# Yelp/nrtsearch

Measured on NVIDIA H100. Metric: BM25 queries/sec (batch 1024, 10M docs), higher is better.
Workload: dtype f32

## Files before the change

### nrtsearch_b200/csrc/probe_kernel.cuh

```cuda
#pragma once
#include "query_eval.cuh"
#include "sort_kernel.cuh"
#include "collect_kernel.cuh"

namespace nrtgpu {
namespace v3 {

__device__ __forceinline__ uint32_t smem_u32(const void* p) { return (uint32_t)__cvta_generic_to_shared(p); }
__device__ __forceinline__ void mbar_init(uint64_t* bar, uint32_t count) {
  asm volatile("mbarrier.init.shared::cta.b64 [%0], %1;" ::"r"(smem_u32(bar)), "r"(count) : "memory");
}
__device__ __forceinline__ void mbar_arrive_expect_tx(uint64_t* bar, uint32_t bytes) {
  asm volatile("mbarrier.arrive.expect_tx.shared::cta.b64 _, [%0], %1;" ::"r"(smem_u32(bar)), "r"(bytes) : "memory");
}
__device__ __forceinline__ bool mbar_try_wait(uint64_t* bar, uint32_t parity) {
  uint32_t ok;
  asm volatile(
      "{\n\t.reg .pred p;\n\tmbarrier.try_wait.parity.shared::cta.b64 p, [%1], %2;\n\tselp.u32 %0, 1, 0, p;\n\t}"
      : "=r"(ok) : "r"(smem_u32(bar)), "r"(parity) : "memory");
  return ok != 0;
}
__device__ __forceinline__ void bulk_g2s(void* dst, const void* src, uint32_t bytes, uint64_t* bar) {
  asm volatile("cp.async.bulk.shared::cluster.global.mbarrier::complete_tx::bytes [%0], [%1], %2, [%3];" ::"r"(smem_u32(dst)),
               "l"(src), "r"(bytes), "r"(smem_u32(bar)) : "memory");
}

__device__ __forceinline__ uint32_t presence4(uint32_t s) {
  return ((s & 0xffu) ? 1u : 0u) | ((s & 0xff00u) ? 2u : 0u) | ((s & 0xff0000u) ? 4u : 0u) | ((s & 0xff000000u) ? 8u : 0u);
}

__device__ __forceinline__ uint32_t expand4(uint32_t m) {
  return ((m & 1u) ? 0xffu : 0u) | ((m & 2u) ? 0xff00u : 0u) | ((m & 4u) ? 0xff0000u : 0u) | ((m & 8u) ? 0xff000000u : 0u);
}

#ifdef NRT_PROBE_KNOCK
#define NRT_KNOCK(bit) ((L.knock & (bit)) != 0)
#else
#define NRT_KNOCK(bit) false
#endif
constexpr int kStageA = 8192;
constexpr int kCtasB = 4, kStageB = 6656;
constexpr int kThreads = 256;
constexpr int kAlign = 16;
constexpr int kPostingPad = 1024;
constexpr int kLongReserve = kT * (kGran + 2 * kAlign);
#ifndef NRT_PROBE_R
#define NRT_PROBE_R 2
#endif
constexpr int kR = NRT_PROBE_R;
constexpr int kCand = 1024;
static_assert(kProbeMaxTopK == kCand / 2, "the probe kernel keeps top_k <= half its candidate buffer");
constexpr int kUbt = 4 * 4 * 4 * 4;
static_assert(sizeof(DevProbeQuery::ubt) == kUbt * sizeof(float), "one bound per tf pattern");
constexpr int kWq = 32 * kR;
constexpr int kProbeStats = 31;
constexpr uint32_t kPiece = 8192;
constexpr uint32_t kTfInexact = 0xFEu;

enum { kAbsent = 0, kLong = 1, kShort = 2, kPlane = 3, kGlobal = 4 };

struct ProbeLaunch {
  DevIndexView ix;
  const DevProbeQuery* pquery;
  const int32_t* work_query;
  const int32_t* work_slice;
  const uint32_t* sbounds;
  unsigned int* work_counter;
  unsigned long long* stats;
  int32_t n_work, n_lists, n_slices, top_k;
  int32_t parts_max;
  int32_t slice_docs;
  int32_t n_gran;
  int64_t threshold;
  int32_t* pruned;
  uint64_t* theta;
  unsigned long long* total_hits;
  uint64_t* slice_keys;
  int32_t* slice_cnt;
  long long deadline_ns;
  unsigned long long* clock0;
  int32_t* timed_out;
  long long terminate_after;
  int32_t* terminated;
  int32_t sort_kind, sort_reverse;
  const uint32_t* sort_codes;
  const uint32_t* sort_missing_code;
  const AggLaunch* aggs;
  const unsigned long long* known_hits;
  int32_t knock;
};

template <int kStageT>
struct alignas(128) ProbeSmemT {
  static constexpr int kStage = kStageT;
  static constexpr int kShortMax = kStageT - kLongReserve;
  static_assert(kShortMax >= 1024, "stage too small");
  int32_t sdocs[kStageT];
  uint8_t sf8[kStageT];
  uint32_t gb[kT][kMaxSliceGran + 4];
  uint64_t cand[kCand];
  uint2 wq[kThreads / 32][kWq];
  DevProbeQuery pq;
  uint64_t stage_bar;
  uint32_t s_ia[kT], s_ib[kT];
  uint32_t s_ra[kT], s_rb[kT];
  int32_t s_sdelta[kT];
  uint32_t s_need[kT];
  uint32_t s_candbelow[kT];
  uint32_t s_cntbefore[kT];
  uint32_t s_pre[kT + 1];
  uint32_t drv_mask, ess_mask, plane_mask, long_mask, short_mask, global_mask;
  int32_t short_total;
  int32_t g1;
  int32_t run_d0, run_d1;
  int32_t staged;
  int wi;
  int skip;
  int cand_count;
  unsigned long long hits0;
  unsigned long long hits_known;
  int theta_dec;
  unsigned long long theta;
  int dbg_theta0;
  int32_t warm_g;
  uint32_t warm_own;
  uint32_t s_candrun[kT], s_cntrun[kT];
  uint32_t run_drv;
};
static_assert(sizeof(ProbeSmemT<kStageA>) <= 232448 / kCtasA - 1024 && sizeof(ProbeSmemT<kStageB>) <= 232448 / kCtasB - 1024, "ProbeSmem exceeds the per-CTA shared memory budget");

__device__ __forceinline__ int32_t seg_first(uint32_t a, uint32_t pbm) { return (int32_t)((a + pbm) & ~(uint32_t)(kAlign - 1)) - (int32_t)pbm; }
__device__ __forceinline__ uint32_t seg_n(uint32_t a, uint32_t b, uint32_t pbm) {
  return b > a ? ((b + pbm + kAlign - 1) & ~(uint32_t)(kAlign - 1)) - ((a + pbm) & ~(uint32_t)(kAlign - 1)) : 0u;
}

template <typename SM>
__device__ __noinline__ bool evaluate_doc(const ProbeLaunch& L, const SM& sm, int32_t doc, uint32_t word, float* out_score) {
  int cur_field = -1;
  uint32_t nb = 1u;
  auto term = [&](const DevClause& c, float* s) {
    uint32_t b = (word >> (8 * c.slot)) & 0xffu;
    if (b == 0) return false;
    if (c.scoring) {
      if (b == kTfInexact && sm.pq.plane[c.slot]) b = (uint32_t)__ldg(sm.pq.plane[c.slot] + doc);
      if (c.field != cur_field) {
        cur_field = c.field;
        const uint8_t* nrm = L.ix.norms[c.field];
        nb = nrm ? (uint32_t)__ldg(nrm + doc) : 1u;
      }
      const float f = (b == 255u) ? exact_freq_slow(L.ix, c, doc) : (float)b;
      *s = bm25_score(c.weight, f, __ldg(&L.ix.caches[c.field * 256 + nb]));
    }
    return true;
  };
  return eval_clauses(L.ix, sm.pq.q, sm.pq.cl, doc, presence4(word), term, out_score);
}

template <typename SM>
__device__ __forceinline__ float score_disjunction(const ProbeLaunch& L, const SM& sm, const uint8_t* norms0, int n_term,
                                                   int32_t doc, uint32_t word) {
  const uint32_t nb = norms0 ? (uint32_t)__ldg(norms0 + doc) : 1u;
  double sum = 0.0;
#pragma unroll
  for (int s = 0; s < kT; ++s) {
    if (s >= n_term) break;
    uint32_t b = (word >> (8 * s)) & 0xffu;
    if (b == 0) continue;
    if (b == kTfInexact && sm.pq.plane[s]) b = (uint32_t)__ldg(sm.pq.plane[s] + doc);
    const float f = (b == 255u) ? exact_freq_slow(L.ix, sm.pq.cl[sm.pq.clause[s]], doc) : (float)b;
    sum += (double)bm25_score(sm.pq.weight[s], f, __ldg(&L.ix.caches[sm.pq.field[s] * 256 + nb]));
  }
  return (float)sum;
}

template <typename SM>
__device__ __noinline__ void flush_candidates(const ProbeLaunch& L, SM& sm, int top_k, uint64_t* g_theta) {
  const long long ts = L.stats ? clock64() : 0ll;
  flush_top_k(sm.cand, sm.cand_count, kCand, top_k, (unsigned long long)sm.theta_dec, g_theta, sm.theta);
  if (L.stats && threadIdx.x == 0) atomicAdd(&L.stats[15], (unsigned long long)(clock64() - ts));
}

template <typename SM>
__device__ __forceinline__ uint32_t probe_smem(const SM& sm, int l, int h, int32_t doc) {
  const int end = h;
  while (l < h) {
    const int mid = (l + h) >> 1;
    if (sm.sdocs[mid] < doc) l = mid + 1; else h = mid;
  }
  return (l < end && sm.sdocs[l] == doc) ? (uint32_t)sm.sf8[l] : 0u;
}
__device__ __noinline__ uint32_t probe_global(const int32_t* docs, const uint8_t* f8, uint32_t l, uint32_t h, int32_t doc) {
  const uint32_t end = h;
  while (l < h) {
    const uint32_t mid = (l + h) >> 1;
    if (__ldg(docs + mid) < doc) l = mid + 1; else h = mid;
  }
  return (l < end && __ldg(docs + l) == doc) ? (uint32_t)__ldg(f8 + l) : 0u;
}

__device__ __forceinline__ uint32_t maxscore_nonessential(const DevProbeQuery& pq, int n_term, unsigned long long theta, bool complete,
                                                          const unsigned long long& hits_known, int64_t threshold) {
  uint32_t ne = 0;
  if (theta != 0ull && (complete || (int64_t)hits_known > threshold)) {
    const float theta_s = key_score(theta);
    for (int a = 0; a < n_term; ++a) {
      if (!(pq.pre[a] < theta_s)) break;
      ne |= 1u << pq.ord[a];
    }
  }
  return ne;
}

template <typename SM>
__device__ __noinline__ void count_role_stats(const ProbeLaunch& L, const SM& sm, int qi, int slice, uint32_t ess_mask,
                                              unsigned long long cyc, unsigned long long driver_postings) {
  const int n_term = sm.pq.q.n_term;
  const uint32_t all = (1u << n_term) - 1u;
  const bool complete = L.threshold >= (int64_t)INT32_MAX;
  const unsigned long long theta = *(volatile unsigned long long*)&L.theta[qi];
  const unsigned long long hits = *(volatile unsigned long long*)&L.total_hits[qi];
  const unsigned long long hits_known = hits > sm.hits_known ? hits : sm.hits_known;
  const uint32_t ne0 = all & ~ess_mask;
  const uint32_t ne1 = maxscore_nonessential(sm.pq, n_term, theta > sm.theta ? theta : sm.theta, complete, hits_known, L.threshold);
  if (sm.dbg_theta0) atomicAdd(&L.stats[19], cyc);
  if ((ne1 & ne0) == ne0 && ne1 != ne0) {
    unsigned long long turned = 0;
    for (int s = 0; s < n_term; ++s) if (((ne1 & ~ne0) >> s) & 1u) turned += sm.s_ib[s] - sm.s_ia[s];
    atomicAdd(&L.stats[22], 1ull); atomicAdd(&L.stats[23], cyc); atomicAdd(&L.stats[24], driver_postings); atomicAdd(&L.stats[25], turned);
    if (slice <= 1) atomicAdd(&L.stats[26 + slice], 1ull);
  }
}

template <bool kSimple, bool kStats, int kCtas, int kStageT, bool kMulti = false>
__global__ void __launch_bounds__(kThreads, kCtas) posting_probe_kernel(const __grid_constant__ ProbeLaunch L) {
  extern __shared__ __align__(128) unsigned char smem_raw[];
  using ProbeSmem = ProbeSmemT<kStageT>;
  constexpr int kStage = kStageT, kShortMax = ProbeSmem::kShortMax;
  ProbeSmem& sm = *reinterpret_cast<ProbeSmem*>(smem_raw);
  const int tid = threadIdx.x;
  const int lane = tid & 31;
  if (tid == 0) {
    mbar_init(&sm.stage_bar, 1);
    asm volatile("fence.mbarrier_init.release.cluster;" ::: "memory");
    asm volatile("fence.proxy.async.shared::cta;" ::: "memory");
  }
  uint32_t stage_parity = 0;
  const int gran_per_slice = L.slice_docs >> kLogGran;
  const int fine = (gran_per_slice + L.parts_max - 1) / L.parts_max;
  const int sb_stride = boundary_entries(L.n_slices, L.parts_max);
  const long long t_cta = kStats ? clock64() : 0ll;

  for (;;) {
    __syncthreads();
    if (tid == 0) {
      const int w = (int)atomicAdd(L.work_counter, 1u);
      sm.wi = w;
      sm.skip = 0;
      if (L.deadline_ns && w < L.n_work && deadline_passed(L.deadline_ns, L.clock0)) {
        sm.skip = 1; L.timed_out[L.work_query[w]] = 1;
      }
    }
    __syncthreads();
    const int wi = sm.wi;
    if (wi >= L.n_work) break;
    if (sm.skip) continue;
    const long long t_start = kStats ? clock64() : 0ll;
    const int qi = L.work_query[wi];
    const int32_t item = L.work_slice[wi];
    const int slice = item_slice(item);
    const int wflags = item_flags(item);
    const bool sweep_warm = (wflags & kItemSweep) != 0;
    const int warm_slot = item_sweep_slot(item);
    const int g_first = slice * gran_per_slice;
    const int g_count = min(gran_per_slice, L.n_gran - g_first);
    const ItemSpan span = item_span(item, g_count, fine, L.parts_max, L.n_slices);
    const int g_lo = span.g_lo, g_hi = span.g_hi;
    {
      constexpr int n16 = (int)((kSimple ? sizeof(DevProbeQuery) : offsetof(DevProbeQuery, ubt)) / 16);
      static_assert(n16 <= kThreads && kThreads == 64 * kT, "one 16-byte piece per thread; 64 threads per slot's granule offsets");
      constexpr int kGbIter = (kMaxSliceGran + 1 + 63) / 64;
      const int gs = tid >> 6, gj = g_lo + (tid & 63);
      const int gran_row = sweep_warm ? -1 : __ldg(&L.pquery[qi].row[gs]);
      uint4 piece = make_uint4(0u, 0u, 0u, 0u);
      if (tid < n16) piece = __ldg(reinterpret_cast<const uint4*>(L.pquery + qi) + tid);
      unsigned long long theta = 0ull, hits0 = 0ull, known = 0ull;
      uint32_t ba = 0, bb = 0, bw = 0, bx = 0;
      int exact_slot = -1;
      if (tid == 0) {
        theta = *(volatile unsigned long long*)&L.theta[qi];
        hits0 = *(volatile unsigned long long*)&L.total_hits[qi];
        if (L.known_hits) known = L.known_hits[qi];
      }
      if (tid >= 32 && tid < 32 + kT) {
        const uint32_t* sb = L.sbounds + ((size_t)qi * kT + (tid - 32)) * sb_stride;
        ba = sb[span.e_lo];
        bb = sb[span.e_hi];
        if (wflags & kItemBehindWarm) bw = sb[boundary_warm_entry(L.n_slices, L.parts_max)];
        if (kSimple && sweep_warm) { exact_slot = __ldg(&L.pquery[qi].warm_slot); bx = sb[boundary_exact_entry(L.n_slices, L.parts_max)]; }
      }
      uint32_t gv[kGbIter];
      const uint32_t* row = L.ix.gran_tab + (size_t)max(gran_row, 0) * (size_t)(L.n_gran + 1) + g_first;
#pragma unroll
      for (int k = 0; k < kGbIter; ++k) gv[k] = (gran_row >= 0 && gj + 64 * k <= g_hi) ? __ldg(row + gj + 64 * k) : 0u;
      if (tid < n16) reinterpret_cast<uint4*>(&sm.pq)[tid] = piece;
      if (tid == 0) {
        sm.cand_count = 0;
        sm.theta = theta; sm.hits0 = hits0; sm.hits_known = known > hits0 ? known : hits0;
        sm.theta_dec = sweep_warm ? 1 : 0;
      }
      if (tid >= 32 && tid < 32 + kT) {
        const int s = tid - 32;
        const uint32_t a = max(ba, bw);
        if (sweep_warm && s == warm_slot) bb = (s == exact_slot) ? bx : min(bb, a + kSweepPostings);
        sm.s_ia[s] = a; sm.s_ib[s] = max(a, bb); sm.s_ra[s] = 0; sm.s_rb[s] = 0; sm.s_sdelta[s] = 0;
      }
#pragma unroll
      for (int k = 0; k < kGbIter; ++k) if (gran_row >= 0 && gj + 64 * k <= g_hi) sm.gb[gs][gj + 64 * k] = gv[k];
    }
    __syncthreads();
    if (L.terminate_after > 0 && (long long)sm.hits0 >= L.terminate_after) {
      if (tid == 0) L.terminated[qi] = 1;
      continue;
    }
    const int n_term = sm.pq.q.n_term;
    if (tid < kT) {
      const int t = tid;
      const uint32_t all = (n_term >= 32) ? 0xffffffffu : ((1u << n_term) - 1u);
      const bool complete = L.threshold >= (int64_t)INT32_MAX;
      const uint32_t ne = (kSimple && !sweep_warm) ? maxscore_nonessential(sm.pq, n_term, sm.theta, complete, sm.hits_known, L.threshold) : 0u;
      uint32_t pm = 0;
      for (int s = 0; s < n_term; ++s) if (sm.pq.kind[s] == kPlane) pm |= 1u << s;
      uint32_t drv, ess;
      int cnt_first = -1;
      const bool exact_warm = kSimple && sm.pq.warm_slot >= 0;
      if (kSimple && sweep_warm) {
        drv = ess = 1u << warm_slot;
        if (t < n_term) { sm.s_candbelow[t] = 0u; sm.s_cntbefore[t] = exact_warm ? 0u : 0xffffffffu; sm.s_need[t] = pm & ~(1u << t); }
      } else if (kSimple) {
        ess = all & ~ne;
        if (complete && ne && !L.ix.live_bits) {
          uint32_t best = 0;
          for (int s = 0; s < n_term; ++s)
            if (((ne & pm) >> s) & 1u) { const uint32_t n = sm.s_ib[s] - sm.s_ia[s]; if (n >= best) { best = n; cnt_first = s; } }
        }
        drv = complete ? (cnt_first >= 0 ? all & ~(1u << cnt_first) : all) : ess;
        if (t < n_term) {
          const uint32_t lower = (1u << t) - 1u;
          const uint32_t first = cnt_first >= 0 ? 1u << cnt_first : 0u;
          const uint32_t below_ess = expand4(ess & lower);
          const uint32_t before_cnt = expand4((lower | first) & ~(1u << t));
          sm.s_candbelow[t] = below_ess;
          sm.s_cntbefore[t] = complete ? before_cnt : below_ess;
          sm.s_need[t] = (complete && !((ess >> t) & 1u)) ? ((lower | first) & ~(1u << t)) : (all & ~(1u << t));
        }
      } else {
        ess = sm.pq.q.dense_driver ? 0u : (sm.pq.q.driver_mask & all);
        drv = ess;
        if (t < n_term) {
          const uint32_t below = expand4(drv & ((1u << t) - 1u));
          sm.s_candbelow[t] = below; sm.s_cntbefore[t] = below;
          sm.s_need[t] = all & ~(1u << t);
        }
      }
      __syncwarp((1u << kT) - 1u);
      if (sweep_warm) {
        if (sm.pq.kind[t] != kPlane && t != warm_slot) sm.pq.kind[t] = kAbsent;
        sm.pq.row[t] = -1;
      }
      __syncwarp((1u << kT) - 1u);
      if (t == 0) {
        if (ne && !complete) L.pruned[qi] = 1;
        if (kSimple) {
          if (exact_warm && sweep_warm) sm.theta_dec = 0;
          const int warm_g = (exact_warm && !sweep_warm) ? sm.pq.warm_gran - g_first : 0;
          sm.warm_g = warm_g;
          sm.warm_own = exact_warm ? 0xffu << (8 * sm.pq.warm_slot) : 0u;
          if (exact_warm && !sweep_warm && warm_g >= g_hi) drv &= ~(1u << sm.pq.warm_slot);
        }
        int st = 0;
        uint32_t lm = 0, shm = 0, gm = 0;
        for (int s = 0; s < n_term; ++s) {
          const int k = sm.pq.kind[s];
          if (k == kLong) lm |= 1u << s;
          else if (k == kShort) {
            const uint32_t a = sm.s_ia[s], b = sm.s_ib[s];
            const int need = (int)seg_n(a, b, sm.pq.pbm[s]);
            if (st + need <= kShortMax) { sm.s_sdelta[s] = st - seg_first(a, sm.pq.pbm[s]); st += need; shm |= 1u << s; }
            else { sm.pq.kind[s] = kGlobal; gm |= 1u << s; }
          }
        }
        if (sweep_warm) { st = 0; lm = 0; shm = 0; gm = 0; }
        sm.short_total = st;
        sm.plane_mask = pm; sm.long_mask = lm; sm.short_mask = shm; sm.global_mask = gm;
        if (cnt_first >= 0 && g_lo < g_hi)
          atomicAdd(&L.total_hits[qi], (unsigned long long)(sm.s_ib[cnt_first] - sm.s_ia[cnt_first]));
        sm.drv_mask = drv; sm.ess_mask = ess;
        if (kStats) {
          sm.dbg_theta0 = kSimple && !sweep_warm && sm.theta == 0ull;
          if (sm.dbg_theta0) { atomicAdd(&L.stats[18], 1ull); if (slice <= 1) atomicAdd(&L.stats[20 + slice], 1ull); }
        }
      }
    }
    __syncthreads();

    const int32_t slice_base = slice * L.slice_docs;
    const uint32_t drv_mask = sm.drv_mask, ess_mask = sm.ess_mask;
    const uint32_t plane_mask = sm.plane_mask, long_mask = sm.long_mask, short_mask = sm.short_mask, global_mask = sm.global_mask;
    unsigned int my_hits = 0;
    unsigned long long dbg_post = 0; unsigned int dbg_runs = 0, dbg_rounds = 0, dbg_flush = 0, dbg_staged = 0, dbg_queued = 0, dbg_admit = 0;
    long long dbg_tflush = 0, dbg_twait = 0;
    const long long t_setup = kStats ? clock64() : 0ll;

    const bool dense = !kSimple && sm.pq.q.dense_driver != 0;
    const uint32_t* live = L.ix.live_bits;
    const uint32_t sort_missing = (!kSimple && L.sort_kind == NRTGPU_SORT_COLUMN) ? *L.sort_missing_code : 0u;
    int g0 = g_lo;
    if (drv_mask == 0u && !dense) g0 = g_hi;
    bool first_run = true;
    while (g0 < g_hi) {
      if (tid == 0) {
        { const unsigned long long g = *(volatile unsigned long long*)&L.theta[qi]; if (g > sm.theta) sm.theta = g; }
        const int cap = kStage - sm.short_total;
        auto fits = [&](int g1) {
          int tot = 0;
#pragma unroll
          for (int s = 0; s < kT; ++s)
            if ((long_mask >> s) & 1u) tot += (int)seg_n(sm.gb[s][g0], sm.gb[s][g1], sm.pq.pbm[s]);
          return tot <= cap;
        };
        int hi = g_hi, lo = g0 + 1;
        uint32_t run_drv = drv_mask;
        if (kSimple) {
          if (g0 < sm.warm_g && sm.warm_g < hi) hi = sm.warm_g;
          const uint32_t own = g0 < sm.warm_g ? sm.warm_own : 0u;
          for (int s = 0; s < kT; ++s) { sm.s_candrun[s] = sm.s_candbelow[s] | own; sm.s_cntrun[s] = sm.s_cntbefore[s] | own; }
          run_drv &= ~presence4(own);
          sm.run_drv = run_drv;
        }
        if (long_mask && hi > lo && !fits(hi)) {
          while (hi - lo > 1) { const int mid = (lo + hi) >> 1; if (fits(mid)) lo = mid; else hi = mid; }
          hi = lo;
        }
        const int g1 = hi;
        sm.g1 = g1;
        const bool whole = (g0 == g_lo && g1 == g_hi);
        const int32_t d0 = slice_base + (g0 << kLogGran);
        const int64_t d1_64 = (int64_t)slice_base + ((int64_t)g1 << kLogGran);
        const int32_t d1 = d1_64 > (int64_t)L.ix.n_docs ? L.ix.n_docs : (int32_t)d1_64;
        sm.run_d0 = d0; sm.run_d1 = d1;
        for (int s = 0; s < n_term; ++s) {
          const int k = sm.pq.kind[s];
          uint32_t a = sm.s_ia[s], b = sm.s_ib[s];
          if (sm.pq.row[s] >= 0) { a = max(a, sm.gb[s][g0]); b = min(b, sm.gb[s][g1]); }
          else if (!whole && b > a) {
            if (k == kShort) {
              if (!first_run) {
                const int base = sm.s_sdelta[s];
                int l = base + (int)a, h = base + (int)b;
                while (l < h) { const int m = (l + h) >> 1; if (sm.sdocs[m] < d0) l = m + 1; else h = m; }
                const uint32_t na = (uint32_t)(l - base);
                h = base + (int)b;
                while (l < h) { const int m = (l + h) >> 1; if (sm.sdocs[m] < d1) l = m + 1; else h = m; }
                a = na; b = (uint32_t)(l - base);
              }
            } else {
              const int32_t* gd = sm.pq.gdocs[s];
              uint32_t l = a, h = b;
              while (l < h) { const uint32_t m = (l + h) >> 1; if (__ldg(gd + m) < d0) l = m + 1; else h = m; }
              const uint32_t na = l;
              h = b;
              while (l < h) { const uint32_t m = (l + h) >> 1; if (__ldg(gd + m) < d1) l = m + 1; else h = m; }
              a = na; b = l;
            }
          }
          if (b < a) b = a;
          sm.s_ra[s] = a; sm.s_rb[s] = b;
        }
        uint32_t total = 0;
        if (first_run)
          for (int s = 0; s < n_term; ++s)
            if ((short_mask >> s) & 1u) total += seg_n(sm.s_ia[s], sm.s_ib[s], sm.pq.pbm[s]) * 5u;
        for (int s = 0; s < n_term; ++s)
          if ((long_mask >> s) & 1u) total += seg_n(sm.s_ra[s], sm.s_rb[s], sm.pq.pbm[s]) * 5u;
        sm.staged = total != 0u;
        if (total) {
          asm volatile("fence.proxy.async.shared::cta;" ::: "memory");
          mbar_arrive_expect_tx(&sm.stage_bar, total);
          auto stage = [&](int s, uint32_t a, uint32_t b, int at) {
            const uint32_t pbm = sm.pq.pbm[s];
            const int32_t f = seg_first(a, pbm);
            const uint32_t n = seg_n(a, b, pbm);
            sm.s_sdelta[s] = at - f;
            const unsigned char* gd = reinterpret_cast<const unsigned char*>(sm.pq.gdocs[s] + f);
            const unsigned char* gf = reinterpret_cast<const unsigned char*>(sm.pq.gf8[s] + f);
            unsigned char* dd = reinterpret_cast<unsigned char*>(&sm.sdocs[at]);
            unsigned char* df = reinterpret_cast<unsigned char*>(&sm.sf8[at]);
            for (uint32_t o = 0; o < n * 4u; o += kPiece) bulk_g2s(dd + o, gd + o, min(kPiece, n * 4u - o), &sm.stage_bar);
            for (uint32_t o = 0; o < n; o += kPiece) bulk_g2s(df + o, gf + o, min(kPiece, n - o), &sm.stage_bar);
            return (int)n;
          };
          if (first_run)
            for (int s = 0; s < n_term; ++s)
              if (((short_mask >> s) & 1u) && sm.s_ib[s] > sm.s_ia[s])
                stage(s, sm.s_ia[s], sm.s_ib[s], sm.s_sdelta[s] + seg_first(sm.s_ia[s], sm.pq.pbm[s]));
          int st = sm.short_total;
          for (int s = 0; s < n_term; ++s)
            if (((long_mask >> s) & 1u) && sm.s_rb[s] > sm.s_ra[s]) st += stage(s, sm.s_ra[s], sm.s_rb[s], st);
        }
        uint32_t pre = 0;
        for (int s = 0; s < kT; ++s) { sm.s_pre[s] = pre; if (s < n_term && ((run_drv >> s) & 1u)) pre += sm.s_rb[s] - sm.s_ra[s]; }
        sm.s_pre[kT] = pre;
      }
      __syncthreads();
      const int g1 = sm.g1;
      if (sm.staged) {
        const long long tw = kStats ? clock64() : 0ll;
        while (!mbar_try_wait(&sm.stage_bar, stage_parity)) {}
        stage_parity ^= 1u;
        if (kStats) dbg_twait += clock64() - tw;
      }
      if (first_run && g1 < g_hi && short_mask) {
        __syncthreads();
        if (tid == 0) {
          const int32_t d0 = slice_base + (g0 << kLogGran);
          const int64_t d1_64 = (int64_t)slice_base + ((int64_t)g1 << kLogGran);
          const int32_t d1 = d1_64 > (int64_t)L.ix.n_docs ? L.ix.n_docs : (int32_t)d1_64;
          for (int s = 0; s < n_term; ++s)
            if (((short_mask >> s) & 1u) && sm.s_ib[s] > sm.s_ia[s]) {
              const int base = sm.s_sdelta[s];
              int l = base + (int)sm.s_ia[s], h = base + (int)sm.s_ib[s];
              while (l < h) { const int m = (l + h) >> 1; if (sm.sdocs[m] < d0) l = m + 1; else h = m; }
              const uint32_t na = (uint32_t)(l - base);
              h = base + (int)sm.s_ib[s];
              while (l < h) { const int m = (l + h) >> 1; if (sm.sdocs[m] < d1) l = m + 1; else h = m; }
              sm.s_ra[s] = na; sm.s_rb[s] = (uint32_t)(l - base);
            }
          uint32_t pre = 0;
          for (int s = 0; s < kT; ++s) { sm.s_pre[s] = pre; if (s < n_term && (((kSimple ? sm.run_drv : drv_mask) >> s) & 1u)) pre += sm.s_rb[s] - sm.s_ra[s]; }
          sm.s_pre[kT] = pre;
        }
        __syncthreads();
      }
      if (kStats) ++dbg_runs;
      const uint32_t n_total = sm.s_pre[kT];
      if (kStats && tid == 0) { dbg_post += n_total; dbg_staged += sm.staged ? 1u : 0u; }
      int ct = 0;
      uint32_t cb = 0;
      uint64_t park = 0ull;
      bool parked = false;
      uint2* const wq = sm.wq[tid >> 5];
      int qn = 0;
      const uint32_t q_req = sm.pq.q.req_term_mask, q_not = sm.pq.q.not_term_mask;
      auto drain = [&](int n_take) -> bool {
        __syncwarp();
        bool fail = false;
        const bool have = lane < n_take;
        const uint2 e = have ? wq[qn - n_take + lane] : make_uint2(0u, 0u);
        qn -= n_take;
        const int32_t d = (int32_t)e.x;
        uint64_t entry = 0ull;
        if (kSimple) {
          if (have) {
            const uint8_t* norms0 = sm.pq.q.single_field >= 0 ? L.ix.norms[sm.pq.q.single_field] : nullptr;
            entry = make_key(score_disjunction(L, sm, norms0, n_term, d, e.y), d);
          }
        } else {
          float score;
          if (have && evaluate_doc(L, sm, d, e.y, &score)) {
            ++my_hits;
            if (L.aggs) agg_collect<kMulti>(*L.aggs, L.ix, qi, d, score);
            if (L.sort_kind == NRTGPU_SORT_RELEVANCE || L.sort_kind == kSortScoreRank) {
              entry = make_key(score, d);
              if (L.sort_kind == kSortScoreRank) entry = make_key(L.sort_reverse ? -score : score, (int32_t)__ldg(L.sort_codes + d));
            } else {
              uint32_t code = 0;
              if (L.sort_kind == NRTGPU_SORT_COLUMN) { code = __ldg(L.sort_codes + d); if (code == 0u) code = sort_missing; }
              entry = ((uint64_t)sort_hi(L.sort_kind, L.sort_reverse, code, d) << 32) | (uint32_t)(~(uint32_t)d);
            }
          }
        }
        const unsigned long long th = sm.theta;
        if (entry > th && !(sm.pq.q.has_after && !(entry < sm.pq.q.after_key)) && !NRT_KNOCK(4)) {
          if (kStats) ++dbg_admit;
          const int p = atomicAdd(&sm.cand_count, 1);
          if (p < kCand) sm.cand[p] = entry;
          else { park = entry; parked = true; fail = true; }
        }
        __syncwarp();
        return fail;
      };
      for (;;) {
        bool full = false;
        if (parked) {
          const int p = atomicAdd(&sm.cand_count, 1);
          if (p < kCand) { sm.cand[p] = park; parked = false; } else full = true;
        }
        full = __any_sync(0xffffffffu, full);
        while (!full && qn >= 32) full = __any_sync(0xffffffffu, drain(32));
        const int ct_end = NRT_KNOCK(8) ? 0 : (dense ? n_term + 1 : n_term);
        while (!full && ct < ct_end) {
          const bool t_dense = ct == n_term;
          const uint32_t n_t = t_dense ? (uint32_t)(sm.run_d1 - sm.run_d0) : ((((kSimple ? sm.run_drv : drv_mask) >> ct) & 1u) ? sm.s_rb[ct] - sm.s_ra[ct] : 0u);
          if (cb >= n_t) { ++ct; cb = 0; continue; }
          const int t = t_dense ? 0 : ct;
          const uint32_t need = t_dense ? ((n_term >= 32) ? 0xffffffffu : ((1u << n_term) - 1u)) : sm.s_need[t];
          const uint32_t need_plane = NRT_KNOCK(1) ? 0u : need & plane_mask, need_long = NRT_KNOCK(2) ? 0u : need & long_mask,
                         need_short = NRT_KNOCK(2) ? 0u : need & short_mask, need_glob = need & global_mask;
          const bool t_staged = !t_dense && (((long_mask | short_mask) >> t) & 1u);
          const bool t_ess = (ess_mask >> t) & 1u;
          const uint32_t candbelow = t_dense ? 0u : (kSimple ? sm.s_candrun[t] : sm.s_candbelow[t]),
                         cntbefore = t_dense ? 0u : (kSimple ? sm.s_cntrun[t] : sm.s_cntbefore[t]);
          const int32_t dense_d0 = sm.run_d0;
          const int32_t* sdoc_t = sm.sdocs + ((int)sm.s_ra[t] + sm.s_sdelta[t]);
          const uint8_t* sf8_t = sm.sf8 + ((int)sm.s_ra[t] + sm.s_sdelta[t]);
          const int32_t* gdoc_t = sm.pq.gdocs[t] + sm.s_ra[t];
          const uint8_t* gf8_t = sm.pq.gf8[t] + sm.s_ra[t];
          const uint32_t tshift = t_dense ? 0u : 8u * (uint32_t)t;
          const int32_t* dptr = t_staged ? sdoc_t : gdoc_t;
          const uint8_t* fptr = t_staged ? sf8_t : gf8_t;
          int32_t nd[kR]; uint32_t nf[kR];
#pragma unroll
          for (int j = 0; j < kR; ++j) {
            const uint32_t x = cb + (uint32_t)(j * kThreads + tid);
            nd[j] = -1; nf[j] = 0;
            if (x < n_t) {
              if (t_dense) nd[j] = dense_d0 + (int32_t)x; else { nd[j] = dptr[x]; nf[j] = fptr[x]; }
            }
          }
          while (!full && cb < n_t) {
            const unsigned long long theta = sm.theta;
            const float theta_s = theta ? key_score(theta) : -INFINITY;
            int32_t doc[kR]; uint32_t word[kR];
            uint32_t pbyte[kR][kT];
#pragma unroll
            for (int j = 0; j < kR; ++j) { doc[j] = nd[j]; word[j] = nf[j] << tshift; }
#pragma unroll
            for (int j = 0; j < kR; ++j) {
              const uint32_t d4 = (uint32_t)max(doc[j], 0) >> 2;
              pbyte[j][0] = 0u; pbyte[j][1] = 0u; pbyte[j][2] = 0u; pbyte[j][3] = 0u;
              if (need_plane & 1u) pbyte[j][0] = (uint32_t)__ldg(sm.pq.plane2[0] + d4);
              if (need_plane & 2u) pbyte[j][1] = (uint32_t)__ldg(sm.pq.plane2[1] + d4);
              if (need_plane & 4u) pbyte[j][2] = (uint32_t)__ldg(sm.pq.plane2[2] + d4);
              if (need_plane & 8u) pbyte[j][3] = (uint32_t)__ldg(sm.pq.plane2[3] + d4);
            }
            {
              const uint32_t nb = cb + (uint32_t)(kR * kThreads);
#pragma unroll
              for (int j = 0; j < kR; ++j) {
                const uint32_t x = nb + (uint32_t)(j * kThreads + tid);
                nd[j] = -1; nf[j] = 0;
                if (x < n_t) {
                  if (t_dense) nd[j] = dense_d0 + (int32_t)x; else { nd[j] = dptr[x]; nf[j] = fptr[x]; }
                }
              }
            }
            if (need_long | need_short | need_glob) {
#pragma unroll
              for (int j = 0; j < kR; ++j) {
                if (doc[j] < 0) continue;
                const int g = (doc[j] - slice_base) >> kLogGran;
#pragma unroll
                for (int u = 0; u < kT; ++u) {
                  uint32_t b = 0;
                  if ((need_long >> u) & 1u) {
                    const uint32_t lo = max(sm.gb[u][g], sm.s_ra[u]), hi = min(sm.gb[u][g + 1], sm.s_rb[u]);
                    if (hi > lo) b = probe_smem(sm, (int)lo + sm.s_sdelta[u], (int)hi + sm.s_sdelta[u], doc[j]);
                  } else if ((need_short >> u) & 1u) {
                    if (sm.s_rb[u] > sm.s_ra[u]) b = probe_smem(sm, (int)sm.s_ra[u] + sm.s_sdelta[u], (int)sm.s_rb[u] + sm.s_sdelta[u], doc[j]);
                  } else if ((need_glob >> u) & 1u) {
                    if (sm.s_rb[u] > sm.s_ra[u]) b = probe_global(sm.pq.gdocs[u], sm.pq.gf8[u], sm.s_ra[u], sm.s_rb[u], doc[j]);
                  }
                  word[j] |= b << (8 * u);
                }
              }
            }
            uint32_t surv_mask = 0;
#pragma unroll
            for (int j = 0; j < kR; ++j) {
              uint32_t v = word[j];
              if (need_plane) {
                const uint32_t raw = pbyte[j][0] | (pbyte[j][1] << 8) | (pbyte[j][2] << 16) | (pbyte[j][3] << 24);
                const uint32_t codes = (raw >> (((uint32_t)max(doc[j], 0) & 3u) * 2u)) & 0x03030303u;
                const uint32_t sat = __vcmpeq4(codes, 0x03030303u);
                v |= (codes & ~sat) | (sat & (kTfInexact * 0x01010101u));
              }
              bool surv = false;
              if (kSimple) {
                if (doc[j] >= 0 && !(live && !((live[doc[j] >> 5] >> (doc[j] & 31)) & 1u))) {
                  if ((v & cntbefore) == 0u) ++my_hits;
                  surv = t_ess && (v & candbelow) == 0u && !(sm.pq.ubt[__dp4a(__vminu4(v, 0x03030303u), 0x40100401u, 0u)] < theta_s);
                }
              } else {
                const uint32_t pres = presence4(v);
                surv = doc[j] >= 0 && (v & candbelow) == 0u && (pres & q_req) == q_req && (pres & q_not) == 0u;
              }
              word[j] = v;
              surv_mask |= surv ? 1u << j : 0u;
            }
#pragma unroll
            for (int j = 0; j < kR; ++j) {
              const bool surv = (surv_mask >> j) & 1u;
              const unsigned bal = __ballot_sync(0xffffffffu, surv);
              if (surv) wq[qn + __popc(bal & ((1u << lane) - 1u))] = make_uint2((uint32_t)doc[j], word[j]);
              qn += __popc(bal);
              if (kStats && lane == 0) dbg_queued += __popc(bal);
              while (!full && qn >= 32) full = __any_sync(0xffffffffu, drain(32));
            }
            cb += kR * kThreads;
            if (kStats && tid == 0) ++dbg_rounds;
          }
        }
        while (!full && qn > 0) full = __any_sync(0xffffffffu, drain(min(qn, 32)));
        __syncthreads();
        if (sm.cand_count <= kCand) break;
        const long long tf = kStats ? clock64() : 0ll;
        flush_candidates(L, sm, L.top_k, &L.theta[qi]);
        if (kStats) dbg_tflush += clock64() - tf;
        if (kStats) ++dbg_flush;
      }
      g0 = g1;
      first_run = false;
      __syncthreads();
    }

    __syncthreads();
    if (sm.cand_count > L.top_k) {
      const long long tf = kStats ? clock64() : 0ll;
      flush_candidates(L, sm, L.top_k, &L.theta[qi]);
      if (kStats) dbg_tflush += clock64() - tf;
      if (kStats) ++dbg_flush;
    }
    const bool lb_warm = kSimple ? sm.theta_dec != 0 : sweep_warm;
    const int keep = lb_warm ? 0 : min(sm.cand_count, L.top_k);
    const int out_list = item_out_list(item, L.parts_max, L.n_lists);
    uint64_t* out = L.slice_keys + ((size_t)qi * L.n_lists + out_list) * L.top_k;
    for (int i = tid; i < keep; i += kThreads) out[i] = sm.cand[i];
    if (tid == 0) L.slice_cnt[(size_t)qi * L.n_lists + out_list] = keep;
    for (int o = 16; o > 0; o >>= 1) my_hits += __shfl_xor_sync(0xffffffffu, my_hits, o);
    if (lane == 0 && my_hits && !lb_warm) atomicAdd(&L.total_hits[qi], (unsigned long long)my_hits);
    if (kStats) {
      for (int o = 16; o > 0; o >>= 1) dbg_admit += __shfl_xor_sync(0xffffffffu, dbg_admit, o);
      if (lane == 0) { atomicAdd(&L.stats[16], (unsigned long long)dbg_queued); atomicAdd(&L.stats[17], (unsigned long long)dbg_admit); }
    }
    if (kStats && tid == 0) {
      const unsigned long long cyc = (unsigned long long)(clock64() - t_start);
      atomicAdd(&L.stats[0], 1ull);
      atomicAdd(&L.stats[1], cyc);
      atomicAdd(&L.stats[2], (unsigned long long)dbg_runs);
      atomicAdd(&L.stats[3], dbg_post);
      atomicAdd(&L.stats[4], (unsigned long long)dbg_flush);
      atomicAdd(&L.stats[5], (unsigned long long)dbg_staged);
      atomicAdd(&L.stats[6], (unsigned long long)(t_setup - t_start));
      atomicAdd(&L.stats[7], (unsigned long long)dbg_rounds);
      atomicMax(&L.stats[8], cyc);
      if (wflags & (kItemWarmDocs | kItemSweep)) { atomicAdd(&L.stats[11], 1ull); atomicAdd(&L.stats[12], cyc); }
      if (sweep_warm && !lb_warm) { atomicAdd(&L.stats[28], 1ull); atomicAdd(&L.stats[29], dbg_post); atomicAdd(&L.stats[30], cyc); }
      atomicAdd(&L.stats[13], (unsigned long long)dbg_tflush); atomicAdd(&L.stats[14], (unsigned long long)dbg_twait);
      if (kSimple && !sweep_warm) count_role_stats(L, sm, qi, item_slice(item), ess_mask, cyc, dbg_post);
    }
  }
  if (kStats && tid == 0) {
    const unsigned long long busy = (unsigned long long)(clock64() - t_cta);
    atomicAdd(&L.stats[9], busy); atomicMax(&L.stats[10], busy);
  }
}

struct SliceBoundsLaunch {
  DevIndexView ix;
  const DevClause* clauses;
  const DevQuery* queries;
  const DevProbeQuery* pquery;
  int32_t nq, n_slices, slice_gran, n_gran, parts_max;
  uint32_t* sbounds;
};

__global__ void slice_bounds_kernel(SliceBoundsLaunch B) {
  const int per_slot = boundary_entries(B.n_slices, B.parts_max);
  const int64_t i = (int64_t)blockIdx.x * blockDim.x + threadIdx.x;
  if (i >= (int64_t)B.nq * kT * per_slot) return;
  const int q = (int)(i / (kT * per_slot)), s = (int)((i / per_slot) % kT), e = (int)(i % per_slot);
  const DevQuery dq = B.queries[q];
  const int64_t gran = e == boundary_exact_entry(B.n_slices, B.parts_max) ? (int64_t)B.pquery[q].warm_gran
                                                                           : boundary_gran(e, B.n_slices, B.parts_max, B.slice_gran, B.n_gran);
  uint32_t out = 0;
  for (int c = 0; c < dq.n_clauses; ++c) {
    const DevClause cl = B.clauses[dq.clause_begin + c];
    if (cl.kind != NRTGPU_TERM || cl.slot != s) continue;
    if (cl.gran_row >= 0) { out = __ldg(B.ix.gran_tab + (size_t)cl.gran_row * (size_t)(B.n_gran + 1) + gran); break; }
    const int64_t target64 = gran << kLogGran;
    const int32_t target = target64 > (int64_t)B.ix.n_docs ? B.ix.n_docs : (int32_t)target64;
    const int32_t* docs = B.ix.post_docs + cl.post_base;
    int lo = 0, hi = cl.n_post;
    while (lo < hi) { const int mid = (lo + hi) >> 1; if (__ldg(docs + mid) < target) lo = mid + 1; else hi = mid; }
    out = (uint32_t)lo;
    break;
  }
  B.sbounds[i] = out;
}

struct ProbeQueryLaunch {
  DevIndexView ix;
  const DevClause* clauses;
  const DevQuery* queries;
  const uint8_t* field_min_norm;
  const int32_t* warm_exact;
  int32_t n_gran;
  DevProbeQuery* out;
};

__global__ void __launch_bounds__(kUbt) probe_query_kernel(ProbeQueryLaunch B) {
  __shared__ DevProbeQuery r;
  __shared__ float uval[kT][2];
  const int qi = blockIdx.x, tid = threadIdx.x;
  const DevQuery dq = B.queries[qi];
  const int ncl = dq.n_clauses, n_term = dq.n_term;
  if (tid == 0) r.q = dq;
  if (tid < kMaxClauses) r.cl[tid] = tid < ncl ? B.clauses[dq.clause_begin + tid] : DevClause{};
  if (tid >= 32 && tid < 32 + kT) {
    const int s = tid - 32;
    r.kind[s] = kAbsent; r.plane[s] = nullptr; r.plane2[s] = nullptr; r.gdocs[s] = nullptr; r.gf8[s] = nullptr;
    r.weight[s] = 0.f; r.ub[s] = 0.f; r.clause[s] = 0; r.field[s] = 0; r.pbm[s] = 0; r.row[s] = -1; r.ord[s] = 0; r.pre[s] = 0.f;
  }
  if (tid == 0) { r.warm_slot = -1; r.warm_gran = 0; r.reserved[0] = r.reserved[1] = 0; }
  __syncthreads();
  if (tid < ncl && r.cl[tid].kind == NRTGPU_TERM) {
    const DevClause& c = r.cl[tid];
    const int s = c.slot;
    r.gdocs[s] = B.ix.post_docs + c.post_base;
    r.gf8[s] = B.ix.post_f8 + c.post_base;
    const bool has_plane = c.plane >= 0 && B.ix.dense_tf != nullptr && B.ix.dense_tf2 != nullptr;
    r.plane[s] = has_plane ? B.ix.dense_tf + (size_t)c.plane * (size_t)B.ix.dense_stride : nullptr;
    r.plane2[s] = has_plane ? B.ix.dense_tf2 + (size_t)c.plane * (size_t)(B.ix.dense_stride >> 2) : nullptr;
    r.kind[s] = has_plane ? kPlane : (c.gran_row >= 0 ? kLong : kShort);
    r.weight[s] = c.weight; r.ub[s] = c.ub; r.clause[s] = tid; r.field[s] = c.field;
    r.pbm[s] = (uint32_t)(c.post_base & (int64_t)(kAlign - 1)); r.row[s] = c.gran_row;
  }
  if (tid >= 64 && tid < 64 + 2 * kT) {
    const int s = (tid - 64) >> 1, c = ((tid - 64) & 1) + 1;
    float u = 0.0f;
    for (int i = 0; i < ncl; ++i)
      if (r.cl[i].kind == NRTGPU_TERM && r.cl[i].slot == s) {
        const uint32_t nbmin = (dq.single_field >= 0 && B.field_min_norm) ? (uint32_t)B.field_min_norm[dq.single_field] : 0u;
        u = bm25_score(r.cl[i].weight, (float)c, __ldg(&B.ix.caches[r.cl[i].field * 256 + nbmin]));
      }
    uval[s][c - 1] = u;
  }
  __syncthreads();
  {
    const int i = tid;
    const int c[kT] = {i & 3, (i >> 2) & 3, (i >> 4) & 3, i >> 6};
    double sum = 0.0;
#pragma unroll
    for (int t = 0; t < kT; ++t) {
      float u = 0.0f;
      if (r.kind[t] != kAbsent && c[t] > 0) u = (c[t] <= 2) ? uval[t][c[t] - 1] : r.weight[t];
      sum += (double)u;
    }
    r.ubt[i] = (float)sum;
  }
  if (tid == 0) {
    int ord[kT]; int n = 0;
    for (int s = 0; s < n_term; ++s) ord[n++] = s;
    for (int a = 1; a < n; ++a) { const int x = ord[a]; int b = a - 1; while (b >= 0 && r.ub[ord[b]] > r.ub[x]) { ord[b + 1] = ord[b]; --b; } ord[b + 1] = x; }
    double pre = 0.0;
    for (int a = 0; a < n; ++a) { pre += (double)r.ub[ord[a]]; r.ord[a] = ord[a]; r.pre[a] = (float)pre; }
    int w = B.warm_exact[qi];
    for (int s = 0; s < n_term; ++s) if (w >= 0 && s != w && r.kind[s] != kPlane) w = -1;
    if (w >= 0) {
      int lo = 0, hi = B.n_gran;
      if (r.row[w] >= 0) {
        const uint32_t* row = B.ix.gran_tab + (size_t)r.row[w] * (size_t)(B.n_gran + 1);
        while (lo < hi) { const int mid = (lo + hi) >> 1; if (__ldg(row + mid) < kSweepPostings) lo = mid + 1; else hi = mid; }
      }
      r.warm_slot = w; r.warm_gran = hi;
    }
  }
  __syncthreads();
  const uint4* src = reinterpret_cast<const uint4*>(&r);
  uint4* dst = reinterpret_cast<uint4*>(B.out + qi);
  for (int i = tid; i < (int)(sizeof(DevProbeQuery) / 16); i += kUbt) dst[i] = src[i];
}

}
}
```

Before: 484,100.

## Software-pipeline plane gathers and compact per-term probe slots in simple path

In the simple scoring path, posting doc/freq loads are now fetched two rounds ahead and the 2-bit plane byte gathers one round ahead, so their global-load latency overlaps the current round's probing and queueing. The per-term probe work is also compacted into at most kT-1 precomputed slots, holding plane pointers or range bounds plus a packed kind/term id, instead of re-testing every term mask per document. The non-simple path keeps the old logic. The deeper prefetch adds register pressure and may lower occupancy. The dense driver case is not handled by the new fetch helper.

New measurement: 523,300 (median of 6 runs). +8.1%, better.

```diff
diff --git a/nrtsearch_b200/csrc/probe_kernel.cuh b/nrtsearch_b200/csrc/probe_kernel.cuh
--- a/nrtsearch_b200/csrc/probe_kernel.cuh
+++ b/nrtsearch_b200/csrc/probe_kernel.cuh
@@ -604,73 +604,163 @@
           if (cb >= n_t) { ++ct; cb = 0; continue; }
           const int t = t_dense ? 0 : ct;
           const uint32_t need = t_dense ? ((n_term >= 32) ? 0xffffffffu : ((1u << n_term) - 1u)) : sm.s_need[t];
-          const uint32_t need_plane = NRT_KNOCK(1) ? 0u : need & plane_mask, need_long = NRT_KNOCK(2) ? 0u : need & long_mask,
-                         need_short = NRT_KNOCK(2) ? 0u : need & short_mask, need_glob = need & global_mask;
           const bool t_staged = !t_dense && (((long_mask | short_mask) >> t) & 1u);
           const bool t_ess = (ess_mask >> t) & 1u;
           const uint32_t candbelow = t_dense ? 0u : (kSimple ? sm.s_candrun[t] : sm.s_candbelow[t]),
                          cntbefore = t_dense ? 0u : (kSimple ? sm.s_cntrun[t] : sm.s_cntbefore[t]);
           const int32_t dense_d0 = sm.run_d0;
-          const int32_t* sdoc_t = sm.sdocs + ((int)sm.s_ra[t] + sm.s_sdelta[t]);
-          const uint8_t* sf8_t = sm.sf8 + ((int)sm.s_ra[t] + sm.s_sdelta[t]);
-          const int32_t* gdoc_t = sm.pq.gdocs[t] + sm.s_ra[t];
-          const uint8_t* gf8_t = sm.pq.gf8[t] + sm.s_ra[t];
           const uint32_t tshift = t_dense ? 0u : 8u * (uint32_t)t;
-          const int32_t* dptr = t_staged ? sdoc_t : gdoc_t;
-          const uint8_t* fptr = t_staged ? sf8_t : gf8_t;
-          int32_t nd[kR]; uint32_t nf[kR];
-#pragma unroll
-          for (int j = 0; j < kR; ++j) {
-            const uint32_t x = cb + (uint32_t)(j * kThreads + tid);
-            nd[j] = -1; nf[j] = 0;
-            if (x < n_t) {
-              if (t_dense) nd[j] = dense_d0 + (int32_t)x; else { nd[j] = dptr[x]; nf[j] = fptr[x]; }
+          constexpr uint32_t kRound = kR * kThreads;
+          constexpr int kP = kT - 1;
+          int32_t doc[kR], nd[kR]; uint32_t df[kR], nf[kR];
+          uint32_t gq[kR][kP];
+          const int sbase = (int)sm.s_ra[t] + sm.s_sdelta[t];
+          const int32_t* gdoc = sm.pq.gdocs[t] + sm.s_ra[t];
+          const uint8_t* gf8 = sm.pq.gf8[t] + sm.s_ra[t];
+          uint64_t pw[kP]; int32_t pd[kP];
+          uint32_t pslot = 0u;
+          int np = 0, n_probe = 0;
+          auto fetch = [&](uint32_t b0, int32_t (&d)[kR], uint32_t (&f)[kR]) {
+#pragma unroll
+            for (int j = 0; j < kR; ++j) {
+              const uint32_t x = b0 + (uint32_t)(j * kThreads + tid);
+              d[j] = -1; f[j] = 0u;
+              if (x < n_t) {
+                if (t_staged) { d[j] = sm.sdocs[sbase + (int)x]; f[j] = sm.sf8[sbase + (int)x]; }
+                else { d[j] = __ldg(gdoc + x); f[j] = __ldg(gf8 + x); }
+              }
+            }
+          };
+          auto gather = [&](const int32_t (&d)[kR], uint32_t (&g)[kR][kP]) {
+#pragma unroll
+            for (int j = 0; j < kR; ++j) {
+              const uint32_t d4 = (uint32_t)max(d[j], 0) >> 2;
+#pragma unroll
+              for (int i = 0; i < kP; ++i) g[j][i] = i < np ? (uint32_t)__ldg(reinterpret_cast<const uint8_t*>(pw[i]) + d4) : 0u;
+            }
+          };
+          const uint32_t need_plane = NRT_KNOCK(1) ? 0u : need & plane_mask, need_long = NRT_KNOCK(2) ? 0u : need & long_mask,
+                         need_short = NRT_KNOCK(2) ? 0u : need & short_mask, need_glob = need & global_mask;
+          const int32_t* dptr = t_staged ? sm.sdocs + sbase : gdoc;
+          const uint8_t* fptr = t_staged ? sm.sf8 + sbase : gf8;
+          if constexpr (kSimple) {
+            uint32_t rest_p = NRT_KNOCK(1) ? 0u : need & plane_mask;
+            uint32_t rest_s = (NRT_KNOCK(2) ? 0u : need & (long_mask | short_mask)) | (need & global_mask);
+            for (int u = 0; u < kT; ++u) if (((rest_s >> u) & 1u) && sm.s_rb[u] <= sm.s_ra[u]) rest_s &= ~(1u << u);
+            np = __popc(rest_p);
+            n_probe = np + __popc(rest_s);
+#pragma unroll
+            for (int i = 0; i < kP; ++i) {
+              pw[i] = 0ull; pd[i] = 0;
+              if (rest_p) {
+                const int u = __ffs(rest_p) - 1;
+                rest_p &= rest_p - 1u;
+                pw[i] = reinterpret_cast<uint64_t>(sm.pq.plane2[u]);
+                pslot |= (uint32_t)u << (8 * i);
+              } else if (rest_s) {
+                const int u = __ffs(rest_s) - 1;
+                rest_s &= rest_s - 1u;
+                const uint32_t kind = ((long_mask >> u) & 1u) ? kLong : (((short_mask >> u) & 1u) ? kShort : kGlobal);
+                pw[i] = (uint64_t)sm.s_ra[u] | ((uint64_t)sm.s_rb[u] << 32);
+                pd[i] = sm.s_sdelta[u];
+                pslot |= ((uint32_t)u | (kind << 2)) << (8 * i);
+              }
+            }
+            fetch(cb, doc, df);
+            gather(doc, gq);
+            fetch(cb + kRound, nd, nf);
+          } else {
+            np = need_plane != 0u;
+#pragma unroll
+            for (int j = 0; j < kR; ++j) {
+              const uint32_t x = cb + (uint32_t)(j * kThreads + tid);
+              nd[j] = -1; nf[j] = 0;
+              if (x < n_t) {
+                if (t_dense) nd[j] = dense_d0 + (int32_t)x; else { nd[j] = dptr[x]; nf[j] = fptr[x]; }
+              }
             }
           }
           while (!full && cb < n_t) {
             const unsigned long long theta = sm.theta;
             const float theta_s = theta ? key_score(theta) : -INFINITY;
-            int32_t doc[kR]; uint32_t word[kR];
+            uint32_t word[kR];
             uint32_t pbyte[kR][kT];
-#pragma unroll
-            for (int j = 0; j < kR; ++j) { doc[j] = nd[j]; word[j] = nf[j] << tshift; }
-#pragma unroll
-            for (int j = 0; j < kR; ++j) {
-              const uint32_t d4 = (uint32_t)max(doc[j], 0) >> 2;
-              pbyte[j][0] = 0u; pbyte[j][1] = 0u; pbyte[j][2] = 0u; pbyte[j][3] = 0u;
-              if (need_plane & 1u) pbyte[j][0] = (uint32_t)__ldg(sm.pq.plane2[0] + d4);
-              if (need_plane & 2u) pbyte[j][1] = (uint32_t)__ldg(sm.pq.plane2[1] + d4);
-              if (need_plane & 4u) pbyte[j][2] = (uint32_t)__ldg(sm.pq.plane2[2] + d4);
-              if (need_plane & 8u) pbyte[j][3] = (uint32_t)__ldg(sm.pq.plane2[3] + d4);
-            }
-            {
-              const uint32_t nb = cb + (uint32_t)(kR * kThreads);
+            uint32_t ngq[kR][kP]; int32_t nnd[kR]; uint32_t nnf[kR];
+            if constexpr (kSimple) {
+              if (cb + kRound < n_t) gather(nd, ngq);
+              else {
+#pragma unroll
+                for (int j = 0; j < kR; ++j)
+#pragma unroll
+                  for (int i = 0; i < kP; ++i) ngq[j][i] = 0u;
+              }
+              fetch(cb + 2 * kRound, nnd, nnf);
+#pragma unroll
+              for (int j = 0; j < kR; ++j) word[j] = df[j] << tshift;
+              if (n_probe > np) {
+#pragma unroll
+                for (int j = 0; j < kR; ++j) {
+                  if (doc[j] < 0) continue;
+                  const int g = (doc[j] - slice_base) >> kLogGran;
+#pragma unroll
+                  for (int i = 0; i < kP; ++i) {
+                    if (i < np || i >= n_probe) continue;
+                    const uint32_t u = (pslot >> (8 * i)) & 3u, kind = (pslot >> (8 * i + 2)) & 7u;
+                    const uint32_t a = (uint32_t)pw[i], b = (uint32_t)(pw[i] >> 32);
+                    uint32_t r = 0;
+                    if (kind == kLong) {
+                      const uint32_t lo = max(sm.gb[u][g], a), hi = min(sm.gb[u][g + 1], b);
+                      if (hi > lo) r = probe_smem(sm, (int)lo + pd[i], (int)hi + pd[i], doc[j]);
+                    } else if (kind == kShort) {
+                      r = probe_smem(sm, (int)a + pd[i], (int)b + pd[i], doc[j]);
+                    } else {
+                      r = probe_global(sm.pq.gdocs[u], sm.pq.gf8[u], a, b, doc[j]);
+                    }
+                    word[j] |= r << (8 * u);
+                  }
+                }
+              }
+            } else {
+#pragma unroll
+              for (int j = 0; j < kR; ++j) { doc[j] = nd[j]; word[j] = nf[j] << tshift; }
 #pragma unroll
               for (int j = 0; j < kR; ++j) {
-                const uint32_t x = nb + (uint32_t)(j * kThreads + tid);
-                nd[j] = -1; nf[j] = 0;
-                if (x < n_t) {
-                  if (t_dense) nd[j] = dense_d0 + (int32_t)x; else { nd[j] = dptr[x]; nf[j] = fptr[x]; }
+                const uint32_t d4 = (uint32_t)max(doc[j], 0) >> 2;
+                pbyte[j][0] = 0u; pbyte[j][1] = 0u; pbyte[j][2] = 0u; pbyte[j][3] = 0u;
+                if (need_plane & 1u) pbyte[j][0] = (uint32_t)__ldg(sm.pq.plane2[0] + d4);
+                if (need_plane & 2u) pbyte[j][1] = (uint32_t)__ldg(sm.pq.plane2[1] + d4);
+                if (need_plane & 4u) pbyte[j][2] = (uint32_t)__ldg(sm.pq.plane2[2] + d4);
+                if (need_plane & 8u) pbyte[j][3] = (uint32_t)__ldg(sm.pq.plane2[3] + d4);
+              }
+              {
+                const uint32_t nb = cb + kRound;
+#pragma unroll
+                for (int j = 0; j < kR; ++j) {
+                  const uint32_t x = nb + (uint32_t)(j * kThreads + tid);
+                  nd[j] = -1; nf[j] = 0;
+                  if (x < n_t) {
+                    if (t_dense) nd[j] = dense_d0 + (int32_t)x; else { nd[j] = dptr[x]; nf[j] = fptr[x]; }
+                  }
                 }
               }
-            }
-            if (need_long | need_short | need_glob) {
-#pragma unroll
-              for (int j = 0; j < kR; ++j) {
-                if (doc[j] < 0) continue;
-                const int g = (doc[j] - slice_base) >> kLogGran;
-#pragma unroll
-                for (int u = 0; u < kT; ++u) {
-                  uint32_t b = 0;
-                  if ((need_long >> u) & 1u) {
-                    const uint32_t lo = max(sm.gb[u][g], sm.s_ra[u]), hi = min(sm.gb[u][g + 1], sm.s_rb[u]);
-                    if (hi > lo) b = probe_smem(sm, (int)lo + sm.s_sdelta[u], (int)hi + sm.s_sdelta[u], doc[j]);
-                  } else if ((need_short >> u) & 1u) {
-                    if (sm.s_rb[u] > sm.s_ra[u]) b = probe_smem(sm, (int)sm.s_ra[u] + sm.s_sdelta[u], (int)sm.s_rb[u] + sm.s_sdelta[u], doc[j]);
-                  } else if ((need_glob >> u) & 1u) {
-                    if (sm.s_rb[u] > sm.s_ra[u]) b = probe_global(sm.pq.gdocs[u], sm.pq.gf8[u], sm.s_ra[u], sm.s_rb[u], doc[j]);
+              if (need_long | need_short | need_glob) {
+#pragma unroll
+                for (int j = 0; j < kR; ++j) {
+                  if (doc[j] < 0) continue;
+                  const int g = (doc[j] - slice_base) >> kLogGran;
+#pragma unroll
+                  for (int u = 0; u < kT; ++u) {
+                    uint32_t b = 0;
+                    if ((need_long >> u) & 1u) {
+                      const uint32_t lo = max(sm.gb[u][g], sm.s_ra[u]), hi = min(sm.gb[u][g + 1], sm.s_rb[u]);
+                      if (hi > lo) b = probe_smem(sm, (int)lo + sm.s_sdelta[u], (int)hi + sm.s_sdelta[u], doc[j]);
+                    } else if ((need_short >> u) & 1u) {
+                      if (sm.s_rb[u] > sm.s_ra[u]) b = probe_smem(sm, (int)sm.s_ra[u] + sm.s_sdelta[u], (int)sm.s_rb[u] + sm.s_sdelta[u], doc[j]);
+                    } else if ((need_glob >> u) & 1u) {
+                      if (sm.s_rb[u] > sm.s_ra[u]) b = probe_global(sm.pq.gdocs[u], sm.pq.gf8[u], sm.s_ra[u], sm.s_rb[u], doc[j]);
+                    }
+                    word[j] |= b << (8 * u);
                   }
-                  word[j] |= b << (8 * u);
                 }
               }
             }
@@ -678,8 +768,14 @@
 #pragma unroll
             for (int j = 0; j < kR; ++j) {
               uint32_t v = word[j];
-              if (need_plane) {
-                const uint32_t raw = pbyte[j][0] | (pbyte[j][1] << 8) | (pbyte[j][2] << 16) | (pbyte[j][3] << 24);
+              if (np) {
+                uint32_t raw = 0u;
+                if constexpr (kSimple) {
+#pragma unroll
+                  for (int i = 0; i < kP; ++i) raw |= gq[j][i] << (8u * ((pslot >> (8 * i)) & 3u));
+                } else {
+                  raw = pbyte[j][0] | (pbyte[j][1] << 8) | (pbyte[j][2] << 16) | (pbyte[j][3] << 24);
+                }
                 const uint32_t codes = (raw >> (((uint32_t)max(doc[j], 0) & 3u) * 2u)) & 0x03030303u;
                 const uint32_t sat = __vcmpeq4(codes, 0x03030303u);
                 v |= (codes & ~sat) | (sat & (kTfInexact * 0x01010101u));
@@ -706,7 +802,15 @@
               if (kStats && lane == 0) dbg_queued += __popc(bal);
               while (!full && qn >= 32) full = __any_sync(0xffffffffu, drain(32));
             }
-            cb += kR * kThreads;
+            if constexpr (kSimple) {
+#pragma unroll
+              for (int j = 0; j < kR; ++j) {
+                doc[j] = nd[j]; df[j] = nf[j]; nd[j] = nnd[j]; nf[j] = nnf[j];
+#pragma unroll
+                for (int i = 0; i < kP; ++i) gq[j][i] = ngq[j][i];
+              }
+            }
+            cb += kRound;
             if (kStats && tid == 0) ++dbg_rounds;
           }
         }
```
